# ojcharles/WeightedLD

Hardware: AMD Instinct MI355X
Metric: LD site-pairs/sec at N=2000 seq × L=20000 var sites; 1/2/4/8 GPU; %HBM roofline (higher is better)
Workload: dtype fp6 (e2m3) weights x fp4 (e2m1) codes on block-scaled MFMA, screen (f32 sums, exact on the rounded weights; rigorous f32 r2 bound over every pair); candidate tiles (0 of 49144): f32 sums in lib.rs's order on f32 MFMA, f32 epilogue

## Files before the change

### weightedld_amd/csrc/capi.hip

```cpp
#include <algorithm>
#include <cmath>
#include <chrono>
#include <condition_variable>
#include <cstdlib>
#include <cstring>
#include <deque>
#include <functional>
#include <mutex>
#include <string>
#include <thread>
#include <vector>

#include "common.hpp"
#include "tile_order.hpp"
#include "window_plan.hpp"
#include "summary_plan.hpp"
#include "heatmap_plan.hpp"
#include "annot_plan.hpp"
#include "matrix_plan.hpp"
#include "blocks_plan.hpp"
#include "partners_plan.hpp"
#include "prune_plan.hpp"
#include "targets_plan.hpp"
#include "kernels.hpp"
// ... 90 lines not shown
    bool opt_fp6_a4 = true;
    int opt_fp6_quick = 1;
    int opt_fp6_three = 1;
    bool opt_fp6_shared = true;
    bool opt_ref_sums = true;
    uint64_t opt_staging_rows = 1ull << 25, opt_host_batch_pairs = 1ull << 31;
    uint64_t opt_target_slots = targets_plan::kDefaultBatchSlots;
    uint64_t opt_partners_bytes = partners_plan::kDefaultBatchBytes;
    uint64_t opt_matrix_bytes = matrix_plan::kDefaultBatchBytes;

    bool loaded = false;
    size_t L = 0, N = 0, LP = 0, NP = 0;
    DevBuf raw, wraw, codes, w_pad, wstats, site_ok, site_map, planes, frag;
    DevBuf rcodes, rw;
    DevBuf w6, f6a, f6b, f6marg;
    DevBuf w4;
    Fp6Screen f6{};
    DevBuf i8a, i8b;
    I8Screen i8s{};
    bool i8img_ok = false;
    bool fp6_tried = false;
    bool fp6_sampled = false;
    bool fp6_ok = false;
    bool fp6_better = false;
    double fp6_rel = 0.0, i8_rel = 0.0;
    bool have_ref = false;
    uint32_t ref_cls = 0;
    size_t NPr = 0;
    DevBuf keep, htab, htab_kept, site_index;
    std::vector<uint64_t> kept_map;
// ... 67 lines not shown
    struct TargetBufs {
        DevBuf slot_site, slot_pos, items, d, dp, r2, mask, tile_pref, slot_cnt, slot_base, guard;
        DevBuf o_t, o_st, o_sp, o_d, o_dp, o_r2;
        std::vector<DevBuf *> all() {
            return {&slot_site, &slot_pos, &items, &d, &dp, &r2, &mask, &tile_pref, &slot_cnt, &slot_base, &guard,
                    &o_t, &o_st, &o_sp, &o_d, &o_dp, &o_r2};
        }
    } tg;
    hipEvent_t ev_tg[2] = {};

    ~wld_ctx() {
        for (wld_ctx *m : members) delete m;
        if (!members.empty()) return;
        (void)hipSetDevice(device);
        if (stream && stream != own_stream) (void)hipStreamSynchronize(stream);
        DevBuf *all[] = {&keep, &htab, &htab_kept, &site_index, &raw, &wraw, &codes, &w_pad, &wstats, &site_ok, &site_map, &planes, &frag, &rcodes, &rw, &w6, &w4, &f6a, &f6b, &f6marg, &i8a, &i8b, &tiles, &cand, &f6_pairs, &fp6_probe_buf,
                         &seg_cnt, &seg_off, &chunk_total, &chunk_base, &counters, &chunk_left, &prog_n, &win_hi, &win_pairs, &sum_buf, &heat_buf, &heat_tiles, &heat_map, &an_buf, &an_tiles, &an_img, &mx_lists, &mx_cnt, &pt_tiles, &pt_stage, &pt_cnt, &pt_csr, &pt_run, &pt_words, &blk_brk, &blk_acc, &blk_map, &blk_tiles, &st_a, &st_b, &st_d,
                         &st_dp, &st_r2, &out_a, &out_b, &out_d, &out_dp, &out_r2};
        for (DevBuf *b : all) release(*b);
        for (DevBuf *b : tg.all()) release(*b);
        for (auto &e : ev_tg)
            if (e) (void)hipEventDestroy(e);
        for (auto &e : ev)
            if (e) (void)hipEventDestroy(e);
        for (auto &e : ev_sum)
            if (e) (void)hipEventDestroy(e);
        for (auto &e : ev_heat)
            if (e) (void)hipEventDestroy(e);
        for (auto &e : ev_an)
            if (e) (void)hipEventDestroy(e);
        for (auto &e : ev_mx)
// ... 78 lines not shown
    for (uint32_t p = 0; p < 4; ++p)
        if (c->wst.plane_mask >> p & 1) top = p;
    const double r8 = (top > 0 ? (double)c->wst.resid[top - 1] : 0.0) + ref_extra_residual(c);
    c->i8_rel = r8 / std::max(std::ldexp((double)c->wst.dsum[top], 8 * (int)top), 1e-300);
    c->f6.a4 = c->opt_fp6_a4 && fp6_codes_fit_fp4(codes.data(), c->N);
    const uint32_t one = c->opt_fp6_shared ? fp6_shared_code(codes.data(), c->N) : 0u;
    c->f6.shared = one != 0u;
    c->f6.wv = (float)fp6_value(one);
    WLD_TRY(ensure(c->w6, c->NP));
    if (c->f6.shared)
        release(c->f6a);
    else
        WLD_TRY(ensure(c->f6a, fp6_a_bytes(c->LP, c->NP, c->f6.a4)));
    WLD_TRY(ensure(c->f6b, fp6_b_bytes(c->LP, c->NP)));
    WLD_TRY(ensure(c->f6marg, 2 * c->LP * sizeof(float)));
    HIP_TRY(hipMemcpyAsync(c->w6.p, codes.data(), c->NP, hipMemcpyHostToDevice, c->stream));
    std::vector<uint8_t> codes4;
    if (c->f6.a4 && !c->f6.shared) {
        codes4.resize(c->NP);
        for (size_t k = 0; k < c->NP; ++k) codes4[k] = (uint8_t)fp6_to_fp4_code(codes[k]);
        WLD_TRY(ensure(c->w4, c->NP));
        HIP_TRY(hipMemcpyAsync(c->w4.p, codes4.data(), c->NP, hipMemcpyHostToDevice, c->stream));
    }
    launch_frag6(ptr<uint8_t>(c->codes), ptr<uint8_t>(c->w6), ptr<uint8_t>(c->f6.a4 ? c->w4 : c->w6), c->f6.a4,
                 c->f6.shared, c->LP, c->NP, c->N, ptr<uint8_t>(c->f6a), ptr<uint8_t>(c->f6b), ptr<float>(c->f6marg),
                 c->stream);
    HIP_TRY(hipGetLastError());
    HIP_TRY(hipStreamSynchronize(c->stream));
    c->f6.b6 = ptr<uint8_t>(c->f6b);
    c->f6.a6 = c->f6.shared ? c->f6.b6 : ptr<uint8_t>(c->f6a);
    c->f6.marg = ptr<float>(c->f6marg);
    c->fp6_ok = true;
    c->fp6_better = c->fp6_rel <= std::max(2.0 * c->i8_rel, 0.02);
    return WLD_OK;
}

int i8img_prepare(wld_ctx *c) {
    uint32_t top = 0;
    for (uint32_t p = 0; p < 4; ++p)
        if (c->plane_mask >> p & 1) top = p;
    WLD_TRY(ensure(c->i8a, i8_a_bytes(c->LP, c->NP)));
    WLD_TRY(ensure(c->i8b, i8_b_bytes(c->LP, c->NP)));
    launch_i8img(ptr<uint8_t>(c->codes), ptr<int8_t>(c->planes) + (size_t)top * c->NP, c->LP, c->NP,
                 ptr<uint8_t>(c->i8a), ptr<uint8_t>(c->i8b), c->stream);
    HIP_TRY(hipGetLastError());
    c->i8s = I8Screen{ptr<uint8_t>(c->i8a), ptr<uint8_t>(c->i8b), top};
// ... 3473 lines not shown
```

### weightedld_amd/csrc/kernels.hpp

```cpp
#pragma once

#include <hip/hip_runtime.h>

#include <cstdint>
#include <vector>

#include "matrix_banded_plan.hpp"
#include "matrix_plan.hpp"
#include "screen_policy.hpp"

namespace wld {

constexpr int kChunk = 256;
constexpr int kTile = 64;
constexpr int kSeqPad = 64;
constexpr int kTilesPerChunk = kChunk / kTile;
constexpr uint32_t kNoTile = 0xFFFFFFFFu;

constexpr uint8_t kCodeIn = 1;
constexpr uint8_t kCodeMaj = 2;

struct OrderArgs {
    uint32_t *st_a, *st_b;
    float *st_d, *st_dp, *st_r2;
// ... 272 lines not shown
constexpr uint32_t kCandidateGrid = 2048;
constexpr uint32_t kRefCandidateGrid = 768;
constexpr uint32_t kRefItemGrid = 1024;
constexpr uint32_t kRefRowsGrid = 2048;

struct Fp6Screen {
    const uint8_t *a6, *b6;
    const float *marg;
    float W6;
    uint32_t NK;
    double R;
    float Tg;
    bool a4;
    bool shared;
    float wv;
};
size_t fp6_a_bytes(size_t LP, size_t NP, bool a4);
size_t fp6_b_bytes(size_t LP, size_t NP);
void launch_frag6(const uint8_t *codes, const uint8_t *w6, const uint8_t *wa, bool a4, bool shared, size_t LP,
                  size_t NP, size_t N, uint8_t *a6, uint8_t *b6, float *marg, hipStream_t s);

struct I8Screen {
    const uint8_t *a8, *b8;
    uint32_t digit_plane;
};
size_t i8_a_bytes(size_t LP, size_t NP);
size_t i8_b_bytes(size_t LP, size_t NP);
void launch_i8img(const uint8_t *codes, const int8_t *digit, size_t LP, size_t NP, uint8_t *a8, uint8_t *b8,
                  hipStream_t s);

struct MfmaLaunch {
    const uint8_t *codes;
    const uint8_t *frag;
// ... 76 lines not shown
```

### weightedld_amd/csrc/pair_common.hpp

```cpp
#pragma once

#include "kernels.hpp"

namespace wld {

#ifndef WLD_EPI_DIVT
#define WLD_EPI_DIVT 1
#endif
__host__ __device__ __forceinline__ double recip_f64(double t, double r0) {
    double r = r0;
    double e = fma(-t, r, 1.0);
    r = fma(r, e, r);
    e = fma(-t, r, 1.0);
    return fma(r, e, r);
}
__host__ __forceinline__ double recip_seed_host(float t) {
    return fabsf(t) < 0x1p-126f ? (double)(1.0f / (t * 0x1p64f)) * 0x1p64 : (double)(1.0f / t);
}
__host__ __device__ __forceinline__ void ld_epilogue(float total_weight, float PA, float PB, float ld3, float &d_out,
                                                     float &dp_out, float &r2_out) {
    float ld_obs0, ld_obs1, ld_obs2, ld_obs3 = ld3;
    float Pa = total_weight - PA;
    float Pb = total_weight - PB;
    ld_obs2 = PA - ld_obs3;
// ... 186 lines not shown
    const float X0lo = p + (a.row + b.col);
    const float cap2 = fminf(fmaf(-2.0f, p, a.Ma2), b.Mb2 - d);
    const float nt = fmaxf(fabsf(fmaf(X0lo, t, q)), fabsf(fmaf(X0lo + cap2, t, q)));
    acc.nt = fmaxf(acc.nt, nt);
    return nt;
}
__host__ __device__ __forceinline__ float f6q_lane_terms(const F6qAcc &acc, const F6qRowMin &a, const F6qColMin &b,
                                                         float thr_c, float E, float &mlo) {
    const float m1 = a.c1 - acc.dmax, m2 = a.rA2 + b.cB2;
    const float m3 = a.rA + b.cB3, m4 = fmaf(-2.0f, acc.pmax, b.c4);
    mlo = fminf(fminf(m1, m2), fminf(m3, m4));
    const float nub = fmaf(2.0f, acc.nt, E);
    return fmaf(nub, nub, -(thr_c * ((m1 * m2) * (m3 * m4))));
}
__host__ __device__ __forceinline__ bool f6q_skip(float t1, float mlo, float mloc) { return t1 <= 0.0f && mlo >= mloc; }
__host__ __device__ __forceinline__ float r2_screen_violation(float T, float A, float B, float AB, float R,
                                                              float thr_c) {
    float E, mloc, t2;
    screen_consts(T, R, E, mloc);
    const float t1 = r2_screen_terms(T, A, B, AB, R, thr_c, E, mloc, t2);
    return fmaxf(t1, t2);
}
__host__ __device__ __forceinline__ bool r2_screen_skip_f32(float T, float A, float B, float AB, float R, float thr) {
    return r2_screen_violation(T, A, B, AB, R, thr * (1.0f - 0x1p-7f)) <= 0.0f;
}
constexpr uint32_t kScreenF32MaxNP = 32768;

__device__ __forceinline__ void glds16(const void *gsrc, uint32_t lds_dst) {
    uint32_t keep;
    asm volatile(
// ... 192 lines not shown
```

### weightedld_amd/csrc/pair_mfma.hip

```cpp
#include <algorithm>
#include <type_traits>
#include <vector>

#include "fp6_pack.hpp"
#include "pair_common.hpp"


namespace wld {

typedef int v4i __attribute__((ext_vector_type(4)));
typedef int v16i __attribute__((ext_vector_type(16)));

bool mfma_supported() { return true; }

namespace {
constexpr int kGroup = 8;
constexpr int kStageCodes = 4096;
constexpr int kDigStage = 128;
constexpr int kMaxPlanes = 4;
constexpr uint32_t kPlanes012 = 0 | (1 << 2) | (2 << 4);
constexpr int kDigGroup = 1024;
template <int NPL>
struct GroupShape {
    static constexpr int kStages = NPL == 1 ? 4 : kGroup;
// ... 682 lines not shown
        const uint32_t e = q >> 3, v8 = e ? (8u + (q & 7u)) << (e - 1) : q;
        miss += (c & kCodeIn) ? 0u : v8;
        minor += (c & (kCodeIn | kCodeMaj)) == kCodeIn ? v8 : 0u;
    }
#pragma unroll
    for (int d = 32; d > 0; d >>= 1) {
        miss += __shfl_xor(miss, d);
        minor += __shfl_xor(minor, d);
    }
    if (lane == 0) {
        marg[2 * (size_t)site] = 0.125f * (float)miss;
        marg[2 * (size_t)site + 1] = 0.125f * (float)minor;
    }
}

namespace {
__device__ __forceinline__ v8i f6_ld24(const uint8_t *p, uint32_t lane) {
    const uint4 x = *reinterpret_cast<const uint4 *>(p + 16 * lane);
    const uint2 y = *reinterpret_cast<const uint2 *>(p + 1024 + 8 * lane);
    asm volatile("" ::: "memory");
    return v8i{(int)x.x, (int)x.y, (int)x.z, (int)x.w, (int)y.x, (int)y.y, 0, 0};
}
__device__ __forceinline__ v8i f6_ldb(const uint8_t *p, uint32_t lane) {
    const uint4 x = *reinterpret_cast<const uint4 *>(p + 16 * lane);
    return v8i{(int)x.x, (int)x.y, (int)x.z, (int)x.w, 0, 0, 0, 0};
}
template <int kFmt>
__device__ __forceinline__ v8i f6_lda(const uint8_t *p, uint32_t lane) {
    if constexpr (kFmt == kF6A4)
        return f6_ldb(p, lane);
// ... 59 lines not shown
        bool cand = false;
#pragma unroll
        for (int i = 0; i < 16; ++i)
            if (!cand) cand = pair_cand(acc, i);
        return cand;
    }
    __device__ __forceinline__ unsigned blocks(const v4f (&acc)[4][2][2]) const {
        unsigned mk = 0;
#pragma unroll
        for (int i = 0; i < 16; ++i)
            if (pair_cand(acc, i)) mk |= 1u << (4 * wq + (i >> 2));
        return mk;
    }
};
template <bool kShared>
__device__ __forceinline__ void f6c_rebuild(v4f (&acc)[4][2][2], const float2 *sA, const float2 *sB, uint32_t wq,
                                            uint32_t lane, float W6, float wv) {
    float col[4], mb[4];
#pragma unroll
    for (int n = 0; n < 4; ++n) {
        const float2 b = sB[(lane & 15) + 16 * n];
        col[n] = f6c_col_term(b.x, b.y);
        mb[n] = b.y;
    }
#pragma unroll
    for (int e = 0; e < 4; ++e) {
        const float2 a = sA[16 * wq + 4 * (lane >> 4) + e];
        const float row = f6c_row_term(W6, a.x), ma2 = 2.0f * a.y;
#pragma unroll
        for (int n = 0; n < 4; ++n) {
            float x0 = acc[n][0][0][e], y0 = acc[n][0][1][e], x1 = acc[n][1][0][e];
            if constexpr (kShared) {
                float y1 = acc[n][1][1][e];
                f6s_direct(x0, y0, x1, y1, row, col[n], ma2, mb[n], wv, 0.5f * wv);
                acc[n][1][1][e] = y1;
            } else {
                f6c_direct(x0, y0, x1, row, col[n], ma2, mb[n]);
            }
            acc[n][0][0][e] = x0;
            acc[n][0][1][e] = y0;
            acc[n][1][0][e] = x1;
        }
    }
}
template <bool kShared>
__device__ __forceinline__ bool f6t_any_doubt(const v4f (&acc)[4][2][2], const F6Epi &ep, const float2 *sA,
                                              const float2 *sB, float W6, float wv) {
    F6tCol cb[4];
#pragma unroll
    for (int n = 0; n < 4; ++n) {
        const float2 b = sB[(ep.lane & 15) + 16 * n];
        cb[n] = f6t_col(b.x, b.y, ep.R2);
    }
    auto terms = [&](const F6tRow &ra, int n, int e, float &mlo) {
        float p = acc[n][0][1][e], s = acc[n][1][0][e], t = acc[n][1][1][e];
        if constexpr (kShared) p *= 0.5f * wv, s *= wv, t *= wv;
        return r2_screen_terms_f6t(p, s, t, ra, cb[n], ep.thr_c, ep.E, mlo);
    };
    if (ep.okA == ~0ull && ep.okB == ~0ull && ep.ta != ep.tb) {
        int worst = -1;
        float mlo_all = INFINITY;
#pragma unroll
        for (int e = 0; e < 4; ++e) {
            const float2 a = sA[16 * ep.wq + 4 * (ep.lane >> 4) + e];
            const F6tRow ra = f6t_row(W6, a.x, a.y, ep.R2);
#pragma unroll
            for (int n = 0; n < 4; ++n) {
                float mlo;
                worst = max(worst, __float_as_int(terms(ra, n, e, mlo)));
                mlo_all = fminf(mlo_all, mlo);
            }
        }
        return worst > 0 || !(mlo_all >= ep.mloc);
    }
    bool doubt = false;
#pragma unroll
    for (int e = 0; e < 4; ++e) {
        const float2 a = sA[16 * ep.wq + 4 * (ep.lane >> 4) + e];
        const F6tRow ra = f6t_row(W6, a.x, a.y, ep.R2);
#pragma unroll
        for (int n = 0; n < 4; ++n) {
            float mlo;
            const float t1 = terms(ra, n, e, mlo);
            if (ep.valid_pair(4 * n + e) && (t1 > 0.0f || !(mlo >= ep.mloc))) doubt = true;
        }
    }
    return doubt;
}
template <bool kShared>
__device__ __forceinline__ bool f6t_quick_skip(const v4f (&acc)[4][2][2], const F6Epi &ep, const float2 *sA,
                                               const F6tCol (&cb)[4], const F6qColMin &cm, float W6, float wv) {
    F6qRowMin rm{INFINITY, INFINITY, INFINITY};
    F6qAcc q;
#pragma unroll
    for (int e = 0; e < 4; ++e) {
        const float2 a = sA[16 * ep.wq + 4 * (ep.lane >> 4) + e];
        const F6tRow ra = f6t_row(W6, a.x, a.y, ep.R2);
        f6q_row_min(rm, ra);
#pragma unroll
        for (int n = 0; n < 4; ++n) {
            float p = acc[n][0][1][e], s = acc[n][1][0][e], t = acc[n][1][1][e];
            if constexpr (kShared) p *= 0.5f * wv, s *= wv, t *= wv;
            f6q_pair(p, s, t, ra, cb[n], q);
            __builtin_amdgcn_sched_barrier(0);
        }
    }
    float mlo;
    const float t1 = f6q_lane_terms(q, rm, cm, ep.thr_c, ep.E, mlo);
    return __ballot(!f6q_skip(t1, mlo, ep.mloc)) == 0;
}
template <bool kShared, bool kQuick>
__device__ __forceinline__ bool f6t_wave_doubt(v4f (&acc)[2][4][2][2], const F6Epi &ep0, const F6Epi &ep1,
                                               const float2 *sA, const float2 *sB, float W6, float wv, uint32_t *full) {
    if constexpr (kQuick) {
        bool full0 = true, full1 = true;
        if (ep0.ta != ep0.tb) {
            F6tCol cb[4];
#pragma unroll
            for (int n = 0; n < 4; ++n) {
                const float2 b = sB[(ep0.lane & 15) + 16 * n];
                cb[n] = f6t_col(b.x, b.y, ep0.R2);
            }
            const F6qColMin cm = f6q_col_min(cb);
            full0 = !f6t_quick_skip<kShared>(acc[0], ep0, sA, cb, cm, W6, wv);
            full1 = !f6t_quick_skip<kShared>(acc[1], ep1, sA, cb, cm, W6, wv);
            if ((full0 || full1) && ep0.lane == 0) atomicAdd(full, (uint32_t)full0 + (uint32_t)full1);
        }
        uint32_t lane = ep0.lane;
        asm volatile("" : "+v"(lane), "+s"(wv)::"memory");
#pragma unroll
        for (int j = 0; j < 2; ++j)
#pragma unroll
            for (int n = 0; n < 4; ++n) asm volatile("" : "+v"(acc[j][n][1][1]));
        F6Epi e0 = ep0, e1 = ep1;
        e0.lane = e1.lane = lane;
        return (full0 && f6t_any_doubt<kShared>(acc[0], e0, sA, sB, W6, wv)) ||
               (full1 && f6t_any_doubt<kShared>(acc[1], e1, sA, sB, W6, wv));
    }
    return f6t_any_doubt<kShared>(acc[0], ep0, sA, sB, W6, wv) ||
           f6t_any_doubt<kShared>(acc[1], ep1, sA, sB, W6, wv);
}
}

template <int kFmt>
__global__ __launch_bounds__(256, 4) void pair_fp6_screen_kernel(const uint8_t *__restrict__ a6,
                                                                  const uint8_t *__restrict__ b6,
                                                                  const float2 *__restrict__ marg, float W6,
                                                                  const uint64_t *__restrict__ ok_bits,
                                                                  const uint32_t *__restrict__ tiles, uint32_t n_tiles,
                                                                  uint32_t NK, uint32_t L, uint32_t n_chunk_rows,
                                                                  float thr, OrderArgs o, ScreenArgs sc, float wv) {
    using F = F6Fmt<kFmt>;
    constexpr int kF6AStage = F::kAStage, kF6ABytes = F::kABytes, kF6Stage = F::kStage;
    __shared__ __attribute__((aligned(16))) uint8_t smem[2 * kF6Stage];
    __shared__ float2 sMarg[2 * kTile];
// ... 75 lines not shown
        screen_verdict((uint32_t)sMask, ta, tb, tid, n_chunk_rows, o, sc);
    } else {
        screen_verdict(0u, ta, tb, tid, n_chunk_rows, o, sc);
    }
}

constexpr uint32_t kF6Single = 0x8000u;

#ifdef WLD_EXP_CLOCK
constexpr uint32_t kF6ClockSlots = 8192;
__device__ unsigned long long gF6Clock[2 * kF6ClockSlots];
extern "C" int wld_debug_f6_clock(unsigned long long *out) {
    return (int)hipMemcpyFromSymbol(out, HIP_SYMBOL(gF6Clock), sizeof(gF6Clock));
}
#endif
template <int kFmt, bool kThree = false, bool kQuick = false>
__global__ __launch_bounds__(256, 3) void pair_fp6_screen2w_kernel(
    const uint8_t *__restrict__ a6, const uint8_t *__restrict__ b6, const float2 *__restrict__ marg, float W6,
    const uint64_t *__restrict__ ok_bits,
    const uint32_t *__restrict__ pairs, uint32_t n_pairs, uint32_t NK, uint32_t L, uint32_t n_chunk_rows, float thr,
    OrderArgs o, ScreenArgs sc, float wv) {
    using F = F6Fmt<kFmt>;
    constexpr int kF6AStage = F::kAStage, kF6ABytes = F::kABytes, kF6PStage = F::kPStage;
    __shared__ __attribute__((aligned(16))) uint8_t smem[2 * kF6PStage];
    __shared__ float2 sMarg[3 * kTile];
    __shared__ unsigned long long sMask[2];
    __shared__ uint32_t sBail, sCand[2];
    __shared__ uint32_t sDoubt[2];
    __shared__ uint32_t sQuickFull;
    static_assert(kThree || !kQuick, "the quick test stands in front of the three-sum test");
    if (!sc.probe && blockIdx.x == 0 && threadIdx.x == 0) *sc.cand_work = 0u;
    const uint32_t tid = threadIdx.x, lane = tid & 63, wave = __builtin_amdgcn_readfirstlane(tid >> 6);
    const uint32_t half = wave >> 1, rp = wave & 1, ltid = tid & 127;
    const uint32_t lds = lds_addr(smem), lane16 = lane * 16;
    const uint32_t ei = sc.probe ? blockIdx.x * sc.probe_stride + blockIdx.x % sc.probe_stride : blockIdx.x;
    const uint32_t entry = ei < n_pairs ? pairs[ei] : kNoTile;
    if (entry == kNoTile) return;
    constexpr int kAPieces = kFmt == kF6A6 ? 3 : kFmt == kF6A4 ? 2 : 1;
    static_assert(kF6AStage == kAPieces * 4096 && kF6BStage == 4096, "five (fp4 A: four, shared: three) pieces per wave and stage");
    struct Src {
// ... 12 lines not shown
        const uint8_t *a = sr.pA + (size_t)kb * kF6AStage;
        const size_t bo = (size_t)kb * kF6BStage;
        glds16_s(a, lane16, gb);
        if (kAPieces > 1) glds16_s(a + 4096, lane16, gb + 4096);
        if (kAPieces > 2) glds16_s(a + 8192, lane16, gb + 8192);
        glds16_s(sr.pB0 + bo, lane16, gb + kF6AStage);
        glds16_s(sr.pB1 + bo, lane16, gb + kF6AStage + kF6BStage);
    };
    const Src cur = src_of(entry);
    issue(cur, 0, 0);
    uint32_t buf = 0;
    {
        const uint32_t ta = entry >> 16, tb0 = entry & 0x7FFFu;
        const bool single = (entry & kF6Single) != 0, idle = single && half;
        const uint32_t tb = tb0 + (idle ? 0u : half);
        if (tid < 3 * kTile) {
            const uint32_t t = tid < kTile ? ta : tb0 + ((tid >= 2 * kTile && !single) ? 1u : 0u);
            sMarg[tid] = marg[t * kTile + (tid & (kTile - 1))];
        }
        if (tid == 0) {
            uint32_t v = 0;
            if (sc.bail) {
                const unsigned cc = __hip_atomic_load(sc.cand_count, __ATOMIC_RELAXED, __HIP_MEMORY_SCOPE_AGENT);
                v = cc > sc.bail ? ((cc & kAbandonBit) ? 2u : 1u) : 0u;
            }
            sBail = v;
        }
        if constexpr (kThree)
            if (tid < 2) sDoubt[tid] = 0u;
        if constexpr (kQuick)
            if (tid == 2) sQuickFull = 0u;
        asm volatile("s_waitcnt lgkmcnt(0)" ::: "memory");
        const uint64_t okA = ok_bits[ta], okB = ok_bits[tb];
// ... 47 lines not shown
        };
#ifdef WLD_EXP_CLOCK
        const unsigned long long ck0 = clock64(), rt0 = wall_clock64();
#endif
        if (!stage(0, std::true_type{})) return;
        for (uint32_t kb = 1; kb < NK; ++kb) stage(kb, std::false_type{});
#ifdef WLD_EXP_CLOCK
        if (tid == 0) {
            gF6Clock[2 * (blockIdx.x % kF6ClockSlots)] = clock64() - ck0;
            gF6Clock[2 * (blockIdx.x % kF6ClockSlots) + 1] = wall_clock64() - rt0;
        }
#endif
        const F6Epi ep0{ta, tb, 2 * rp, lane, okA, okB, 2.0f * sc.Rf, thr * (1.0f - 0x1p-7f), sc.E, sc.mloc};
        const F6Epi ep1{ta, tb, 2 * rp + 1, lane, okA, okB, 2.0f * sc.Rf, thr * (1.0f - 0x1p-7f), sc.E, sc.mloc};
        if constexpr (kThree) {
            const float2 *sB = sMarg + kTile * (1 + half);
            const bool doubt =
                !idle && f6t_wave_doubt<F::kShared, kQuick>(acc, ep0, ep1, sMarg, sB, W6, wv, &sQuickFull);
            if (doubt) sDoubt[half] = 1u;
            __syncthreads();
            if constexpr (kQuick) {
                unsigned *const cnt = sc.probe ? sc.probe + 3 : sc.rechecked ? sc.rechecked + 1 : nullptr;
                if (tid == 0 && cnt && sQuickFull) atomicAdd(cnt, sQuickFull);
            }
#ifdef WLD_EXP_ZERO_IMG
            const bool again = (sDoubt[0] | sDoubt[1]) == 0x5EEDu;
#else
            const bool again = (sDoubt[0] | sDoubt[1]) != 0;
#endif
            if (!again) {
                if (sc.probe) {
                    if (ltid == 0 && !idle) atomicAdd(sc.probe + 1, 1u);
                } else if (!idle) {
// ... 19 lines not shown
                } else {
                    ai0 = f6_lda<kFmt>(g + aoff, lane);
                    ai1 = f6_lda<kFmt>(g + aoff + kF6ABytes, lane);
                }
#pragma unroll
                for (int n = 0; n < 4; ++n) {
                    const v8i b = f6_ldb(g + boff + n * kF6BBytes, lane);
                    acc[0][n][0][0] = f6_mfma<F::kCbsz>(ai0, b, acc[0][n][0][0]);
                    acc[1][n][0][0] = f6_mfma<F::kCbsz>(ai1, b, acc[1][n][0][0]);
                }
                asm volatile("s_waitcnt lgkmcnt(0)" ::: "memory");
                buf ^= 1;
            }
        }
        if (!idle) {
            f6c_rebuild<F::kShared>(acc[0], sMarg, sMarg + kTile * (1 + half), 2 * rp, lane, W6, wv);
            f6c_rebuild<F::kShared>(acc[1], sMarg, sMarg + kTile * (1 + half), 2 * rp + 1, lane, W6, wv);
        }
        const bool cand = !idle && (ep0.any(acc[0]) || ep1.any(acc[1]));
        if (cand) sCand[half] = 1u;
        __syncthreads();
#ifdef WLD_EXP_ZERO_IMG
        const bool mine = sCand[half] == 0x5EEDu;
#else
        const bool mine = sCand[half] != 0;
#endif
        if (sc.probe) {
            if (ltid == 0 && !idle) {
                if (mine) atomicAdd(sc.probe, 1u);
                atomicAdd(sc.probe + 1, 1u);
            }
            return;
// ... 159 lines not shown

void launch_frag6(const uint8_t *codes, const uint8_t *w6, const uint8_t *wa, bool a4, bool shared, size_t LP,
                  size_t NP, size_t N, uint8_t *a6, uint8_t *b6, float *marg, hipStream_t s) {
    const size_t n = LP / 16 * ((NP + 127) / 128) * 64;
    const dim3 grid((unsigned)((n + 255) / 256));
    if (shared)
        hipLaunchKernelGGL(frag6_shared_kernel, grid, dim3(256), 0, s, codes, (uint32_t)LP, (uint32_t)NP, (uint32_t)N, b6);
    else if (a4)
        hipLaunchKernelGGL(frag6_kernel<true>, grid, dim3(256), 0, s, codes, wa, (uint32_t)LP, (uint32_t)NP, a6, b6);
    else
        hipLaunchKernelGGL(frag6_kernel<false>, grid, dim3(256), 0, s, codes, wa, (uint32_t)LP, (uint32_t)NP, a6, b6);
    hipLaunchKernelGGL(fp6_marginals_kernel, dim3((unsigned)((LP + 3) / 4)), dim3(256), 0, s, codes, w6, (uint32_t)LP,
                       (uint32_t)NP, marg);
}

template <int MODE>
__global__ __launch_bounds__(256, 2) void pair_mfma_rows_kernel(const uint8_t *__restrict__ codes,
                                                                 const int8_t *__restrict__ planes,
                                                                 const uint64_t *__restrict__ ok_bits,
                                                                 const uint32_t *__restrict__ tiles, uint32_t L,
                                                                 uint32_t NP, uint32_t n_chunk_rows, float thr,
                                                                 int shift, OrderArgs o, DenseArgs dn, ScreenArgs sc) {
    __shared__ unsigned long long sBits[kTile];
    __shared__ uint32_t sRowBase[kTile];
    const uint32_t tile = tiles[blockIdx.x];
    if (tile == kNoTile) return;
    const uint32_t ta = tile >> 16, tb = tile & 0xFFFFu;
    const uint32_t tid = threadIdx.x, lane = tid & 63, wave = tid >> 6;
    const uint32_t wa = wave >> 1, wb = wave & 1, r = lane & 31, h = lane >> 5;
    Acc32<3> acc;
// ... 95 lines not shown
        v.tile_work = sc.cand_work;
        v.tile_buckets = sc.cand_buckets;
        v.bucket_cap = sc.cand_cap;
        v.rb_items = sc.rb_items != 0;
        v.scan = sc.scan;
        launch_pair_valu(v, o, nullptr, s);
        return;
    }
    const uint32_t grid = std::min<uint32_t>(m.n_tiles, kCandidateGrid);
    launch_lds_planes<kModePrefilter, true>(n, m, ok_bits, m.cand_list, 0, m.cand_count, grid, idx, o, dn, sc, s);
}
}

namespace {
void fp6_screen_args(const MfmaLaunch &m, ScreenArgs &sc) {
    sc.R = std::ceil(m.fp6->R * 32.0) / 32.0;
    sc.Rf = (float)sc.R;
    sc.f32 = 2;
    screen_consts(m.fp6->Tg, 2.0f * sc.Rf, sc.E, sc.mloc);
}
template <int kFmt>
void launch_fp6_screen_fmt(const MfmaLaunch &m, const uint64_t *ok_bits, const OrderArgs &o, const ScreenArgs &sc,
                           uint32_t stride, hipStream_t s) {
    if (m.f6_pairs && m.fp6_three && m.fp6_quick) {
        hipLaunchKernelGGL((pair_fp6_screen2w_kernel<kFmt, true, true>), dim3((m.f6_n_pairs + stride - 1) / stride),
                           dim3(256), 0, s, m.fp6->a6, m.fp6->b6, reinterpret_cast<const float2 *>(m.fp6->marg),
                           m.fp6->W6, ok_bits, m.f6_pairs, m.f6_n_pairs, m.fp6->NK, m.L, m.n_chunk_rows, m.thr, o, sc,
                           m.fp6->wv);
    } else if (m.f6_pairs && m.fp6_three) {
        hipLaunchKernelGGL((pair_fp6_screen2w_kernel<kFmt, true>), dim3((m.f6_n_pairs + stride - 1) / stride),
                           dim3(256), 0, s, m.fp6->a6, m.fp6->b6, reinterpret_cast<const float2 *>(m.fp6->marg),
                           m.fp6->W6, ok_bits, m.f6_pairs, m.f6_n_pairs, m.fp6->NK, m.L, m.n_chunk_rows, m.thr, o, sc,
                           m.fp6->wv);
    } else if (m.f6_pairs) {
        hipLaunchKernelGGL(pair_fp6_screen2w_kernel<kFmt>, dim3((m.f6_n_pairs + stride - 1) / stride), dim3(256), 0, s,
                           m.fp6->a6, m.fp6->b6, reinterpret_cast<const float2 *>(m.fp6->marg), m.fp6->W6, ok_bits,
                           m.f6_pairs, m.f6_n_pairs, m.fp6->NK, m.L, m.n_chunk_rows,
                           m.thr, o, sc, m.fp6->wv);
    } else {
        hipLaunchKernelGGL(pair_fp6_screen_kernel<kFmt>, dim3((m.n_tiles + stride - 1) / stride), dim3(256), 0, s,
                           m.fp6->a6, m.fp6->b6, reinterpret_cast<const float2 *>(m.fp6->marg), m.fp6->W6, ok_bits,
                           m.tiles, m.n_tiles, m.fp6->NK, m.L, m.n_chunk_rows, m.thr,
                           o, sc, m.fp6->wv);
    }
}
void launch_fp6_screen(const MfmaLaunch &m, const uint64_t *ok_bits, const OrderArgs &o, const ScreenArgs &sc,
                       uint32_t stride, hipStream_t s) {
    if (m.fp6->shared)
        launch_fp6_screen_fmt<kF6Shared>(m, ok_bits, o, sc, stride, s);
    else if (m.fp6->a4)
        launch_fp6_screen_fmt<kF6A4>(m, ok_bits, o, sc, stride, s);
    else
        launch_fp6_screen_fmt<kF6A6>(m, ok_bits, o, sc, stride, s);
// ... 127 lines not shown
```

Before: 508.7 billion.

## Precompute per-site fp6 screen records and use count units for shared weights

Adds a one-time kernel that precomputes the per-site row and column screen terms and their group minima into a device records buffer. The three-sum fp6 screen kernel now stages these records into shared memory instead of recomputing f6t_row/f6t_col from marginals in every tile epilogue. When all weights share one power-of-two value, a new count-unit variant rescales the records and constants so the per-pair wv multiplies disappear. The cost is extra global and LDS traffic per tile entry (6400 bytes staged), plus more kernel instantiations to maintain.

```diff
diff --git a/weightedld_amd/csrc/capi.hip b/weightedld_amd/csrc/capi.hip
--- a/weightedld_amd/csrc/capi.hip
+++ b/weightedld_amd/csrc/capi.hip
@@ -128,6 +128,7 @@
     DevBuf raw, wraw, codes, w_pad, wstats, site_ok, site_map, planes, frag;
     DevBuf rcodes, rw;
     DevBuf w6, f6a, f6b, f6marg;
+    DevBuf f6rec;
     DevBuf w4;
     Fp6Screen f6{};
     DevBuf i8a, i8b;
@@ -225,7 +226,7 @@
         if (!members.empty()) return;
         (void)hipSetDevice(device);
         if (stream && stream != own_stream) (void)hipStreamSynchronize(stream);
-        DevBuf *all[] = {&keep, &htab, &htab_kept, &site_index, &raw, &wraw, &codes, &w_pad, &wstats, &site_ok, &site_map, &planes, &frag, &rcodes, &rw, &w6, &w4, &f6a, &f6b, &f6marg, &i8a, &i8b, &tiles, &cand, &f6_pairs, &fp6_probe_buf,
+        DevBuf *all[] = {&keep, &htab, &htab_kept, &site_index, &raw, &wraw, &codes, &w_pad, &wstats, &site_ok, &site_map, &planes, &frag, &rcodes, &rw, &w6, &w4, &f6a, &f6b, &f6marg, &f6rec, &i8a, &i8b, &tiles, &cand, &f6_pairs, &fp6_probe_buf,
                          &seg_cnt, &seg_off, &chunk_total, &chunk_base, &counters, &chunk_left, &prog_n, &win_hi, &win_pairs, &sum_buf, &heat_buf, &heat_tiles, &heat_map, &an_buf, &an_tiles, &an_img, &mx_lists, &mx_cnt, &pt_tiles, &pt_stage, &pt_cnt, &pt_csr, &pt_run, &pt_words, &blk_brk, &blk_acc, &blk_map, &blk_tiles, &st_a, &st_b, &st_d,
                          &st_dp, &st_r2, &out_a, &out_b, &out_d, &out_dp, &out_r2};
         for (DevBuf *b : all) release(*b);
@@ -334,6 +335,7 @@
         WLD_TRY(ensure(c->f6a, fp6_a_bytes(c->LP, c->NP, c->f6.a4)));
     WLD_TRY(ensure(c->f6b, fp6_b_bytes(c->LP, c->NP)));
     WLD_TRY(ensure(c->f6marg, 2 * c->LP * sizeof(float)));
+    WLD_TRY(ensure(c->f6rec, fp6_rec_bytes(c->LP)));
     HIP_TRY(hipMemcpyAsync(c->w6.p, codes.data(), c->NP, hipMemcpyHostToDevice, c->stream));
     std::vector<uint8_t> codes4;
     if (c->f6.a4 && !c->f6.shared) {
@@ -346,10 +348,12 @@
                  c->f6.shared, c->LP, c->NP, c->N, ptr<uint8_t>(c->f6a), ptr<uint8_t>(c->f6b), ptr<float>(c->f6marg),
                  c->stream);
     HIP_TRY(hipGetLastError());
+    c->f6.marg = ptr<float>(c->f6marg);
+    launch_fp6_records(c->f6, c->LP, c->f6rec.p, c->stream);
+    HIP_TRY(hipGetLastError());
     HIP_TRY(hipStreamSynchronize(c->stream));
     c->f6.b6 = ptr<uint8_t>(c->f6b);
     c->f6.a6 = c->f6.shared ? c->f6.b6 : ptr<uint8_t>(c->f6a);
-    c->f6.marg = ptr<float>(c->f6marg);
     c->fp6_ok = true;
     c->fp6_better = c->fp6_rel <= std::max(2.0 * c->i8_rel, 0.02);
     return WLD_OK;
diff --git a/weightedld_amd/csrc/kernels.hpp b/weightedld_amd/csrc/kernels.hpp
--- a/weightedld_amd/csrc/kernels.hpp
+++ b/weightedld_amd/csrc/kernels.hpp
@@ -310,9 +310,13 @@
     bool a4;
     bool shared;
     float wv;
+    const void *rec;
+    bool counts;
 };
 size_t fp6_a_bytes(size_t LP, size_t NP, bool a4);
 size_t fp6_b_bytes(size_t LP, size_t NP);
+size_t fp6_rec_bytes(size_t LP);
+void launch_fp6_records(Fp6Screen &f, size_t LP, void *rec, hipStream_t s);
 void launch_frag6(const uint8_t *codes, const uint8_t *w6, const uint8_t *wa, bool a4, bool shared, size_t LP,
                   size_t NP, size_t N, uint8_t *a6, uint8_t *b6, float *marg, hipStream_t s);
 
diff --git a/weightedld_amd/csrc/pair_common.hpp b/weightedld_amd/csrc/pair_common.hpp
--- a/weightedld_amd/csrc/pair_common.hpp
+++ b/weightedld_amd/csrc/pair_common.hpp
@@ -224,6 +224,54 @@
     return fmaf(nub, nub, -(thr_c * ((m1 * m2) * (m3 * m4))));
 }
 __host__ __device__ __forceinline__ bool f6q_skip(float t1, float mlo, float mloc) { return t1 <= 0.0f && mlo >= mloc; }
+template <bool kTwice>
+__host__ __device__ __forceinline__ float f6q_pair1(float ap, float s, float t, float ma2, float row, float mb,
+                                                    float col, float cW, F6qAcc &acc) {
+    const float d = s - t;
+    acc.dmax = fmaxf(acc.dmax, d);
+    acc.pmax = fmaxf(acc.pmax, ap);
+    const float rc = row + col;
+    const float y0 = kTwice ? fmaf(-0.5f, ap, mb) : mb - ap;
+    const float lo = kTwice ? fmaf(0.5f, ap, rc) : ap + rc;
+    const float hi = kTwice ? fmaf(-0.5f, ap, cW) : cW - ap;
+    const float q = -((ma2 - s) * y0);
+    const float nt = fmaxf(fabsf(fmaf(lo, t, q)), fabsf(fmaf(hi, t, q)));
+    acc.nt = fmaxf(acc.nt, nt);
+    return nt;
+}
+template <bool kTwice>
+__host__ __device__ __forceinline__ void f6q_pmax(F6qAcc &acc) {
+    if (kTwice) acc.pmax *= 0.5f;
+}
+struct alignas(8) F6RowRec {
+    F6tRow a;
+};
+struct alignas(16) F6ColRec {
+    F6tCol b;
+    float cW, pad;
+};
+struct alignas(16) F6MinRec {
+    float x, y, z, pad;
+};
+__host__ __device__ __forceinline__ F6RowRec f6_row_rec(float W6, float Ma, float ma, float R2, float inv) {
+    const F6tRow a = f6t_row(W6, Ma, ma, R2);
+    return F6RowRec{{a.rA * inv, a.rA2 * inv, a.c1 * inv, a.Ma2 * inv, a.ma2 * inv, a.row * inv}};
+}
+__host__ __device__ __forceinline__ F6ColRec f6_col_rec(float W6, float Mb, float mb, float R2, float inv) {
+    const F6tCol b = f6t_col(Mb, mb, R2);
+    return F6ColRec{{b.cB2 * inv, b.cB3 * inv, b.c4 * inv, b.Mb2 * inv, b.mb * inv, b.col * inv},
+                    fmaf(2.0f, W6, b.col) * inv, 0.0f};
+}
+__host__ __device__ __forceinline__ F6MinRec f6_row_min_rec(const F6RowRec (&r)[4]) {
+    F6qRowMin m{INFINITY, INFINITY, INFINITY};
+    for (int e = 0; e < 4; ++e) f6q_row_min(m, r[e].a);
+    return F6MinRec{m.c1, m.rA2, m.rA, 0.0f};
+}
+__host__ __device__ __forceinline__ F6MinRec f6_col_min_rec(const F6ColRec (&c)[4]) {
+    const F6tCol b[4] = {c[0].b, c[1].b, c[2].b, c[3].b};
+    const F6qColMin m = f6q_col_min(b);
+    return F6MinRec{m.cB2, m.cB3, m.c4, 0.0f};
+}
 __host__ __device__ __forceinline__ float r2_screen_violation(float T, float A, float B, float AB, float R,
                                                               float thr_c) {
     float E, mloc, t2;
diff --git a/weightedld_amd/csrc/pair_mfma.hip b/weightedld_amd/csrc/pair_mfma.hip
--- a/weightedld_amd/csrc/pair_mfma.hip
+++ b/weightedld_amd/csrc/pair_mfma.hip
@@ -720,6 +720,26 @@
     }
 }
 
+__global__ __launch_bounds__(256) void fp6_records_kernel(const float2 *__restrict__ marg, float W6, float R2, float inv,
+                                                           uint32_t LP, F6RowRec *__restrict__ row,
+                                                           F6ColRec *__restrict__ col, F6MinRec *__restrict__ rmin,
+                                                           F6MinRec *__restrict__ cmin) {
+    const uint32_t s = blockIdx.x * 256 + threadIdx.x;
+    if (s >= LP) return;
+    auto row_of = [&](uint32_t i) { return f6_row_rec(W6, marg[i].x, marg[i].y, R2, inv); };
+    auto col_of = [&](uint32_t i) { return f6_col_rec(W6, marg[i].x, marg[i].y, R2, inv); };
+    row[s] = row_of(s);
+    col[s] = col_of(s);
+    if ((s & 3) == 0) {
+        const F6RowRec r[4] = {row_of(s), row_of(s + 1), row_of(s + 2), row_of(s + 3)};
+        rmin[s >> 2] = f6_row_min_rec(r);
+    }
+    if ((s & (kTile - 1)) < 16) {
+        const F6ColRec c[4] = {col_of(s), col_of(s + 16), col_of(s + 32), col_of(s + 48)};
+        cmin[(s >> 6) * 16 + (s & 15)] = f6_col_min_rec(c);
+    }
+}
+
 namespace {
 __device__ __forceinline__ v8i f6_ld24(const uint8_t *p, uint32_t lane) {
     const uint4 x = *reinterpret_cast<const uint4 *>(p + 16 * lane);
@@ -809,6 +829,24 @@
     }
 };
 template <bool kShared>
+__device__ __forceinline__ void f6c_rebuild_row(v4f (&acc)[4][2][2], int e, float row, float ma2,
+                                                const float (&col)[4], const float (&mb)[4], float wv) {
+#pragma unroll
+    for (int n = 0; n < 4; ++n) {
+        float x0 = acc[n][0][0][e], y0 = acc[n][0][1][e], x1 = acc[n][1][0][e];
+        if constexpr (kShared) {
+            float y1 = acc[n][1][1][e];
+            f6s_direct(x0, y0, x1, y1, row, col[n], ma2, mb[n], wv, 0.5f * wv);
+            acc[n][1][1][e] = y1;
+        } else {
+            f6c_direct(x0, y0, x1, row, col[n], ma2, mb[n]);
+        }
+        acc[n][0][0][e] = x0;
+        acc[n][0][1][e] = y0;
+        acc[n][1][0][e] = x1;
+    }
+}
+template <bool kShared>
 __device__ __forceinline__ void f6c_rebuild(v4f (&acc)[4][2][2], const float2 *sA, const float2 *sB, uint32_t wq,
                                             uint32_t lane, float W6, float wv) {
     float col[4], mb[4];
@@ -821,35 +859,41 @@
 #pragma unroll
     for (int e = 0; e < 4; ++e) {
         const float2 a = sA[16 * wq + 4 * (lane >> 4) + e];
-        const float row = f6c_row_term(W6, a.x), ma2 = 2.0f * a.y;
-#pragma unroll
-        for (int n = 0; n < 4; ++n) {
-            float x0 = acc[n][0][0][e], y0 = acc[n][0][1][e], x1 = acc[n][1][0][e];
-            if constexpr (kShared) {
-                float y1 = acc[n][1][1][e];
-                f6s_direct(x0, y0, x1, y1, row, col[n], ma2, mb[n], wv, 0.5f * wv);
-                acc[n][1][1][e] = y1;
-            } else {
-                f6c_direct(x0, y0, x1, row, col[n], ma2, mb[n]);
-            }
-            acc[n][0][0][e] = x0;
-            acc[n][0][1][e] = y0;
-            acc[n][1][0][e] = x1;
-        }
-    }
-}
-template <bool kShared>
-__device__ __forceinline__ bool f6t_any_doubt(const v4f (&acc)[4][2][2], const F6Epi &ep, const float2 *sA,
-                                              const float2 *sB, float W6, float wv) {
+        f6c_rebuild_row<kShared>(acc, e, f6c_row_term(W6, a.x), 2.0f * a.y, col, mb, wv);
+    }
+}
+struct F6Site {
+    const F6RowRec *row;
+    const F6ColRec *col;
+    const F6MinRec *rmin, *cmin;
+};
+template <bool kShared, bool kCounts>
+__device__ __forceinline__ void f6c_rebuild_rec(v4f (&acc)[4][2][2], const F6Site &st, uint32_t wq, uint32_t lane,
+                                                float wv) {
+    float col[4], mb[4];
+#pragma unroll
+    for (int n = 0; n < 4; ++n) {
+        const F6tCol &b = st.col[(lane & 15) + 16 * n].b;
+        col[n] = kCounts ? b.col * wv : b.col;
+        mb[n] = kCounts ? b.mb * wv : b.mb;
+    }
+#pragma unroll
+    for (int e = 0; e < 4; ++e) {
+        const F6tRow &a = st.row[16 * wq + 4 * (lane >> 4) + e].a;
+        f6c_rebuild_row<kShared>(acc, e, kCounts ? a.row * wv : a.row, kCounts ? a.ma2 * wv : a.ma2, col, mb, wv);
+    }
+}
+template <bool kShared, bool kCounts>
+__device__ __forceinline__ bool f6t_any_doubt(const v4f (&acc)[4][2][2], const F6Epi &ep, const F6Site &st, float wv) {
     F6tCol cb[4];
 #pragma unroll
-    for (int n = 0; n < 4; ++n) {
-        const float2 b = sB[(ep.lane & 15) + 16 * n];
-        cb[n] = f6t_col(b.x, b.y, ep.R2);
-    }
+    for (int n = 0; n < 4; ++n) cb[n] = st.col[(ep.lane & 15) + 16 * n].b;
     auto terms = [&](const F6tRow &ra, int n, int e, float &mlo) {
         float p = acc[n][0][1][e], s = acc[n][1][0][e], t = acc[n][1][1][e];
-        if constexpr (kShared) p *= 0.5f * wv, s *= wv, t *= wv;
+        if constexpr (kCounts)
+            p *= 0.5f;
+        else if constexpr (kShared)
+            p *= 0.5f * wv, s *= wv, t *= wv;
         return r2_screen_terms_f6t(p, s, t, ra, cb[n], ep.thr_c, ep.E, mlo);
     };
     if (ep.okA == ~0ull && ep.okB == ~0ull && ep.ta != ep.tb) {
@@ -857,8 +901,7 @@
         float mlo_all = INFINITY;
 #pragma unroll
         for (int e = 0; e < 4; ++e) {
-            const float2 a = sA[16 * ep.wq + 4 * (ep.lane >> 4) + e];
-            const F6tRow ra = f6t_row(W6, a.x, a.y, ep.R2);
+            const F6tRow ra = st.row[16 * ep.wq + 4 * (ep.lane >> 4) + e].a;
 #pragma unroll
             for (int n = 0; n < 4; ++n) {
                 float mlo;
@@ -871,8 +914,7 @@
     bool doubt = false;
 #pragma unroll
     for (int e = 0; e < 4; ++e) {
-        const float2 a = sA[16 * ep.wq + 4 * (ep.lane >> 4) + e];
-        const F6tRow ra = f6t_row(W6, a.x, a.y, ep.R2);
+        const F6tRow ra = st.row[16 * ep.wq + 4 * (ep.lane >> 4) + e].a;
 #pragma unroll
         for (int n = 0; n < 4; ++n) {
             float mlo;
@@ -882,43 +924,48 @@
     }
     return doubt;
 }
-template <bool kShared>
-__device__ __forceinline__ bool f6t_quick_skip(const v4f (&acc)[4][2][2], const F6Epi &ep, const float2 *sA,
-                                               const F6tCol (&cb)[4], const F6qColMin &cm, float W6, float wv) {
-    F6qRowMin rm{INFINITY, INFINITY, INFINITY};
+struct F6qCol {
+    float mb, col, cW;
+};
+template <bool kShared, bool kCounts>
+__device__ __forceinline__ bool f6t_quick_skip(const v4f (&acc)[4][2][2], const F6Epi &ep, const F6Site &st,
+                                               const F6qCol (&cb)[4], const F6qColMin &cm, float wv) {
+    const uint32_t grp = 4 * ep.wq + (ep.lane >> 4);
     F6qAcc q;
 #pragma unroll
     for (int e = 0; e < 4; ++e) {
-        const float2 a = sA[16 * ep.wq + 4 * (ep.lane >> 4) + e];
-        const F6tRow ra = f6t_row(W6, a.x, a.y, ep.R2);
-        f6q_row_min(rm, ra);
+        const F6tRow &ra = st.row[4 * grp + e].a;
+        const float ma2 = ra.ma2, row = ra.row;
 #pragma unroll
         for (int n = 0; n < 4; ++n) {
             float p = acc[n][0][1][e], s = acc[n][1][0][e], t = acc[n][1][1][e];
-            if constexpr (kShared) p *= 0.5f * wv, s *= wv, t *= wv;
-            f6q_pair(p, s, t, ra, cb[n], q);
+            if constexpr (kShared && !kCounts) p *= 0.5f * wv, s *= wv, t *= wv;
+            f6q_pair1<kCounts>(p, s, t, ma2, row, cb[n].mb, cb[n].col, cb[n].cW, q);
             __builtin_amdgcn_sched_barrier(0);
         }
     }
+    f6q_pmax<kCounts>(q);
+    const F6MinRec r = st.rmin[grp];
     float mlo;
-    const float t1 = f6q_lane_terms(q, rm, cm, ep.thr_c, ep.E, mlo);
+    const float t1 = f6q_lane_terms(q, F6qRowMin{r.x, r.y, r.z}, cm, ep.thr_c, ep.E, mlo);
     return __ballot(!f6q_skip(t1, mlo, ep.mloc)) == 0;
 }
-template <bool kShared, bool kQuick>
+template <bool kShared, bool kQuick, bool kCounts>
 __device__ __forceinline__ bool f6t_wave_doubt(v4f (&acc)[2][4][2][2], const F6Epi &ep0, const F6Epi &ep1,
-                                               const float2 *sA, const float2 *sB, float W6, float wv, uint32_t *full) {
+                                               const F6Site &st, float wv, uint32_t *full) {
     if constexpr (kQuick) {
         bool full0 = true, full1 = true;
         if (ep0.ta != ep0.tb) {
-            F6tCol cb[4];
+            F6qCol cb[4];
 #pragma unroll
             for (int n = 0; n < 4; ++n) {
-                const float2 b = sB[(ep0.lane & 15) + 16 * n];
-                cb[n] = f6t_col(b.x, b.y, ep0.R2);
-            }
-            const F6qColMin cm = f6q_col_min(cb);
-            full0 = !f6t_quick_skip<kShared>(acc[0], ep0, sA, cb, cm, W6, wv);
-            full1 = !f6t_quick_skip<kShared>(acc[1], ep1, sA, cb, cm, W6, wv);
+                const F6ColRec &b = st.col[(ep0.lane & 15) + 16 * n];
+                cb[n] = F6qCol{b.b.mb, b.b.col, b.cW};
+            }
+            const F6MinRec c = st.cmin[ep0.lane & 15];
+            const F6qColMin cm{c.x, c.y, c.z};
+            full0 = !f6t_quick_skip<kShared, kCounts>(acc[0], ep0, st, cb, cm, wv);
+            full1 = !f6t_quick_skip<kShared, kCounts>(acc[1], ep1, st, cb, cm, wv);
             if ((full0 || full1) && ep0.lane == 0) atomicAdd(full, (uint32_t)full0 + (uint32_t)full1);
         }
         uint32_t lane = ep0.lane;
@@ -929,11 +976,10 @@
             for (int n = 0; n < 4; ++n) asm volatile("" : "+v"(acc[j][n][1][1]));
         F6Epi e0 = ep0, e1 = ep1;
         e0.lane = e1.lane = lane;
-        return (full0 && f6t_any_doubt<kShared>(acc[0], e0, sA, sB, W6, wv)) ||
-               (full1 && f6t_any_doubt<kShared>(acc[1], e1, sA, sB, W6, wv));
-    }
-    return f6t_any_doubt<kShared>(acc[0], ep0, sA, sB, W6, wv) ||
-           f6t_any_doubt<kShared>(acc[1], ep1, sA, sB, W6, wv);
+        return (full0 && f6t_any_doubt<kShared, kCounts>(acc[0], e0, st, wv)) ||
+               (full1 && f6t_any_doubt<kShared, kCounts>(acc[1], e1, st, wv));
+    }
+    return f6t_any_doubt<kShared, kCounts>(acc[0], ep0, st, wv) || f6t_any_doubt<kShared, kCounts>(acc[1], ep1, st, wv);
 }
 }
 
@@ -1039,16 +1085,36 @@
     return (int)hipMemcpyFromSymbol(out, HIP_SYMBOL(gF6Clock), sizeof(gF6Clock));
 }
 #endif
-template <int kFmt, bool kThree = false, bool kQuick = false>
+struct F6Recs {
+    const F6ColRec *col;
+    const F6RowRec *row;
+    const F6MinRec *rmin, *cmin;
+    float inv;
+};
+constexpr int kF6SiteCol = 0, kF6SiteRow = 2 * kTile * sizeof(F6ColRec), kF6SiteRmin = kF6SiteRow + kTile * sizeof(F6RowRec),
+              kF6SiteCmin = kF6SiteRmin + kTile / 4 * sizeof(F6MinRec),
+              kF6SiteBytes = kF6SiteCmin + 2 * 16 * sizeof(F6MinRec);
+static_assert(sizeof(F6ColRec) == 32 && sizeof(F6RowRec) == 24 && sizeof(F6MinRec) == 16 && kF6SiteBytes == 6400 &&
+                  kF6SiteRow % 16 == 0 && kF6SiteRmin % 16 == 0,
+              "the entry's records are staged as 400 16-byte pieces");
+__device__ __forceinline__ F6Site f6_site_of(const uint8_t *site, uint32_t half) {
+    return F6Site{reinterpret_cast<const F6RowRec *>(site + kF6SiteRow),
+                  reinterpret_cast<const F6ColRec *>(site + kF6SiteCol) + kTile * half,
+                  reinterpret_cast<const F6MinRec *>(site + kF6SiteRmin),
+                  reinterpret_cast<const F6MinRec *>(site + kF6SiteCmin) + 16 * half};
+}
+template <int kFmt, bool kThree = false, bool kQuick = false, bool kCounts = false>
 __global__ __launch_bounds__(256, 3) void pair_fp6_screen2w_kernel(
     const uint8_t *__restrict__ a6, const uint8_t *__restrict__ b6, const float2 *__restrict__ marg, float W6,
     const uint64_t *__restrict__ ok_bits,
     const uint32_t *__restrict__ pairs, uint32_t n_pairs, uint32_t NK, uint32_t L, uint32_t n_chunk_rows, float thr,
-    OrderArgs o, ScreenArgs sc, float wv) {
+    OrderArgs o, ScreenArgs sc, float wv, F6Recs rec) {
     using F = F6Fmt<kFmt>;
     constexpr int kF6AStage = F::kAStage, kF6ABytes = F::kABytes, kF6PStage = F::kPStage;
+    static_assert(!kCounts || (kThree && F::kShared), "count units: the shared image's three-sum tests");
     __shared__ __attribute__((aligned(16))) uint8_t smem[2 * kF6PStage];
-    __shared__ float2 sMarg[3 * kTile];
+    __shared__ __attribute__((aligned(kThree ? 16 : 8))) uint8_t sSite[kThree ? kF6SiteBytes : 3 * kTile * sizeof(float2)];
+    const float2 *const sMarg = reinterpret_cast<const float2 *>(sSite);
     __shared__ unsigned long long sMask[2];
     __shared__ uint32_t sBail, sCand[2];
     __shared__ uint32_t sDoubt[2];
@@ -1091,9 +1157,20 @@
         const uint32_t ta = entry >> 16, tb0 = entry & 0x7FFFu;
         const bool single = (entry & kF6Single) != 0, idle = single && half;
         const uint32_t tb = tb0 + (idle ? 0u : half);
-        if (tid < 3 * kTile) {
+        if constexpr (kThree) {
+            const uint32_t tb1 = tb0 + (single ? 0u : 1u);
+            uint4 *const dst = reinterpret_cast<uint4 *>(sSite);
+            dst[tid] = reinterpret_cast<const uint4 *>(rec.col + (tid < 128 ? tb0 : tb1) * kTile)[tid & 127];
+            if (tid < 96)
+                dst[kF6SiteRow / 16 + tid] = reinterpret_cast<const uint4 *>(rec.row + ta * kTile)[tid];
+            else if (tid < 112)
+                dst[kF6SiteRmin / 16 + (tid - 96)] = reinterpret_cast<const uint4 *>(rec.rmin + ta * (kTile / 4))[tid - 96];
+            else if (tid < 144)
+                dst[kF6SiteCmin / 16 + (tid - 112)] =
+                    reinterpret_cast<const uint4 *>(rec.cmin + (tid < 128 ? tb0 : tb1) * 16)[tid & 15];
+        } else if (tid < 3 * kTile) {
             const uint32_t t = tid < kTile ? ta : tb0 + ((tid >= 2 * kTile && !single) ? 1u : 0u);
-            sMarg[tid] = marg[t * kTile + (tid & (kTile - 1))];
+            reinterpret_cast<float2 *>(sSite)[tid] = marg[t * kTile + (tid & (kTile - 1))];
         }
         if (tid == 0) {
             uint32_t v = 0;
@@ -1171,9 +1248,12 @@
         const F6Epi ep0{ta, tb, 2 * rp, lane, okA, okB, 2.0f * sc.Rf, thr * (1.0f - 0x1p-7f), sc.E, sc.mloc};
         const F6Epi ep1{ta, tb, 2 * rp + 1, lane, okA, okB, 2.0f * sc.Rf, thr * (1.0f - 0x1p-7f), sc.E, sc.mloc};
         if constexpr (kThree) {
-            const float2 *sB = sMarg + kTile * (1 + half);
+            const F6Site st = f6_site_of(sSite, half);
+            F6Epi t0 = ep0, t1 = ep1;
+            t0.E = t1.E = kCounts ? sc.E * rec.inv * rec.inv : sc.E;
+            t0.mloc = t1.mloc = kCounts ? sc.mloc * rec.inv : sc.mloc;
             const bool doubt =
-                !idle && f6t_wave_doubt<F::kShared, kQuick>(acc, ep0, ep1, sMarg, sB, W6, wv, &sQuickFull);
+                !idle && f6t_wave_doubt<F::kShared, kQuick, kCounts>(acc, t0, t1, st, wv, &sQuickFull);
             if (doubt) sDoubt[half] = 1u;
             __syncthreads();
             if constexpr (kQuick) {
@@ -1223,8 +1303,14 @@
             }
         }
         if (!idle) {
-            f6c_rebuild<F::kShared>(acc[0], sMarg, sMarg + kTile * (1 + half), 2 * rp, lane, W6, wv);
-            f6c_rebuild<F::kShared>(acc[1], sMarg, sMarg + kTile * (1 + half), 2 * rp + 1, lane, W6, wv);
+            if constexpr (kThree) {
+                const F6Site st = f6_site_of(sSite, half);
+                f6c_rebuild_rec<F::kShared, kCounts>(acc[0], st, 2 * rp, lane, wv);
+                f6c_rebuild_rec<F::kShared, kCounts>(acc[1], st, 2 * rp + 1, lane, wv);
+            } else {
+                f6c_rebuild<F::kShared>(acc[0], sMarg, sMarg + kTile * (1 + half), 2 * rp, lane, W6, wv);
+                f6c_rebuild<F::kShared>(acc[1], sMarg, sMarg + kTile * (1 + half), 2 * rp + 1, lane, W6, wv);
+            }
         }
         const bool cand = !idle && (ep0.any(acc[0]) || ep1.any(acc[1]));
         if (cand) sCand[half] = 1u;
@@ -1414,6 +1500,33 @@
                        (uint32_t)NP, marg);
 }
 
+namespace {
+double fp6_screen_R(const Fp6Screen &f) { return std::ceil(f.R * 32.0) / 32.0; }
+F6Recs fp6_recs_of(const void *rec, size_t LP, float inv) {
+    const uint8_t *p = static_cast<const uint8_t *>(rec);
+    F6Recs r;
+    r.col = reinterpret_cast<const F6ColRec *>(p);
+    r.row = reinterpret_cast<const F6RowRec *>(p + LP * sizeof(F6ColRec));
+    r.rmin = reinterpret_cast<const F6MinRec *>(p + LP * (sizeof(F6ColRec) + sizeof(F6RowRec)));
+    r.cmin = r.rmin + LP / 4;
+    r.inv = inv;
+    return r;
+}
+}
+size_t fp6_rec_bytes(size_t LP) {
+    return LP * (sizeof(F6ColRec) + sizeof(F6RowRec)) + (LP / 4 + LP / kTile * 16) * sizeof(F6MinRec);
+}
+void launch_fp6_records(Fp6Screen &f, size_t LP, void *rec, hipStream_t s) {
+    int e = 0;
+    f.counts = f.shared && std::frexp(f.wv, &e) == 0.5f;
+    f.rec = rec;
+    const F6Recs r = fp6_recs_of(rec, LP, f.counts ? 1.0f / f.wv : 1.0f);
+    hipLaunchKernelGGL(fp6_records_kernel, dim3((unsigned)((LP + 255) / 256)), dim3(256), 0, s,
+                       reinterpret_cast<const float2 *>(f.marg), f.W6, 2.0f * (float)fp6_screen_R(f), r.inv,
+                       (uint32_t)LP, const_cast<F6RowRec *>(r.row), const_cast<F6ColRec *>(r.col),
+                       const_cast<F6MinRec *>(r.rmin), const_cast<F6MinRec *>(r.cmin));
+}
+
 template <int MODE>
 __global__ __launch_bounds__(256, 2) void pair_mfma_rows_kernel(const uint8_t *__restrict__ codes,
                                                                  const int8_t *__restrict__ planes,
@@ -1539,7 +1652,7 @@
 
 namespace {
 void fp6_screen_args(const MfmaLaunch &m, ScreenArgs &sc) {
-    sc.R = std::ceil(m.fp6->R * 32.0) / 32.0;
+    sc.R = fp6_screen_R(*m.fp6);
     sc.Rf = (float)sc.R;
     sc.f32 = 2;
     screen_consts(m.fp6->Tg, 2.0f * sc.Rf, sc.E, sc.mloc);
@@ -1547,21 +1660,25 @@
 template <int kFmt>
 void launch_fp6_screen_fmt(const MfmaLaunch &m, const uint64_t *ok_bits, const OrderArgs &o, const ScreenArgs &sc,
                            uint32_t stride, hipStream_t s) {
+    const bool counts = kFmt == kF6Shared && m.fp6->counts;
+    const F6Recs rec = fp6_recs_of(m.fp6->rec, m.LP, counts ? 1.0f / m.fp6->wv : 1.0f);
+    auto pairs = [&](auto kernel) {
+        hipLaunchKernelGGL(kernel, dim3((m.f6_n_pairs + stride - 1) / stride), dim3(256), 0, s, m.fp6->a6, m.fp6->b6,
+                           reinterpret_cast<const float2 *>(m.fp6->marg), m.fp6->W6, ok_bits, m.f6_pairs, m.f6_n_pairs,
+                           m.fp6->NK, m.L, m.n_chunk_rows, m.thr, o, sc, m.fp6->wv, rec);
+    };
     if (m.f6_pairs && m.fp6_three && m.fp6_quick) {
-        hipLaunchKernelGGL((pair_fp6_screen2w_kernel<kFmt, true, true>), dim3((m.f6_n_pairs + stride - 1) / stride),
-                           dim3(256), 0, s, m.fp6->a6, m.fp6->b6, reinterpret_cast<const float2 *>(m.fp6->marg),
-                           m.fp6->W6, ok_bits, m.f6_pairs, m.f6_n_pairs, m.fp6->NK, m.L, m.n_chunk_rows, m.thr, o, sc,
-                           m.fp6->wv);
+        if constexpr (kFmt == kF6Shared) {
+            if (counts) return pairs(pair_fp6_screen2w_kernel<kFmt, true, true, true>);
+        }
+        pairs(pair_fp6_screen2w_kernel<kFmt, true, true>);
     } else if (m.f6_pairs && m.fp6_three) {
-        hipLaunchKernelGGL((pair_fp6_screen2w_kernel<kFmt, true>), dim3((m.f6_n_pairs + stride - 1) / stride),
-                           dim3(256), 0, s, m.fp6->a6, m.fp6->b6, reinterpret_cast<const float2 *>(m.fp6->marg),
-                           m.fp6->W6, ok_bits, m.f6_pairs, m.f6_n_pairs, m.fp6->NK, m.L, m.n_chunk_rows, m.thr, o, sc,
-                           m.fp6->wv);
+        if constexpr (kFmt == kF6Shared) {
+            if (counts) return pairs(pair_fp6_screen2w_kernel<kFmt, true, false, true>);
+        }
+        pairs(pair_fp6_screen2w_kernel<kFmt, true>);
     } else if (m.f6_pairs) {
-        hipLaunchKernelGGL(pair_fp6_screen2w_kernel<kFmt>, dim3((m.f6_n_pairs + stride - 1) / stride), dim3(256), 0, s,
-                           m.fp6->a6, m.fp6->b6, reinterpret_cast<const float2 *>(m.fp6->marg), m.fp6->W6, ok_bits,
-                           m.f6_pairs, m.f6_n_pairs, m.fp6->NK, m.L, m.n_chunk_rows,
-                           m.thr, o, sc, m.fp6->wv);
+        pairs(pair_fp6_screen2w_kernel<kFmt>);
     } else {
         hipLaunchKernelGGL(pair_fp6_screen_kernel<kFmt>, dim3((m.n_tiles + stride - 1) / stride), dim3(256), 0, s,
                            m.fp6->a6, m.fp6->b6, reinterpret_cast<const float2 *>(m.fp6->marg), m.fp6->W6, ok_bits,
```

Result: faster. 520.6 billion, median of 6 (+2.3%).
